# 331658260/Drone-YOLO

Measured on AMD Instinct MI355X. Metric: images/sec @640x640 Drone-YOLO-s, higher is better.
Workload: dtype fp16; 1 GPU; Drone-YOLO-s (yolov8s-p2-repvgg.yaml, nc=10) inference 640x640: layout+forward+decode+NMS, inputs resident in HBM; fp16 storage / fp32 accumulate (BASELINE config 2 names bf16: bf16 storage fails the IoU >= 0.999 bar - 0.995 - so the headline runs the 16-bit format that meets it; same MFMA rate, same bytes); batch_per_gpu=256, global_batch=256, parallelism=batch-split x1, no collective, hipgraph=True, streams=2, max_det=300

## Files before the change

### drone-yolo_amd/_lib.py

```python
from __future__ import annotations

import ctypes as C
import os

_HERE = os.path.dirname(os.path.abspath(__file__))
LIB_PATH = os.path.join(_HERE, "lib", "libdyolo.so")

DY_BF16, DY_F16, DY_F32, DY_FP8, DY_F16X2 = 0, 1, 2, 3, 4
DY_ACT_NONE, DY_ACT_SILU, DY_ACT_SILU_L2E = 0, 1, 2
DY_MAX_LEVELS = 8
DY_WLAYOUT_ROWS, DY_WLAYOUT_HALO3X3, DY_WLAYOUT_FRAG1X1 = 0, 1, 2

_vp, _i32, _f32, _i64 = C.c_void_p, C.c_int32, C.c_float, C.c_int64


class PackJob(C.Structure):
    _fields_ = [("w", C.c_void_p), ("s_co", C.c_int64), ("s_ci", C.c_int64), ("s_r", C.c_int64), ("s_q", C.c_int64),
                ("cout", C.c_int32), ("cin", C.c_int32), ("ksize", C.c_int32), ("transpose_flip", C.c_int32), ("cin_logical", C.c_int32),
                ("w_layout", C.c_int32), ("dst", C.c_void_p), ("dst_elems", C.c_int64)]


class ConvDesc(C.Structure):

    _fields_ = [
        ("x", _vp), ("w", _vp), ("bias", _vp), ("residual", _vp), ("y", _vp),
        ("batch", _i32), ("h", _i32), ("w_in", _i32), ("cin", _i32), ("ld_x", _i32),
        ("ho", _i32), ("wo", _i32), ("cout", _i32), ("ld_y", _i32), ("ld_res", _i32),
        ("ksize", _i32), ("stride", _i32), ("pad", _i32),
        ("groups", _i32), ("act", _i32), ("dtype", _i32), ("out_f32", _i32),
        ("k_pad", _i32), ("cout_pad", _i32), ("up2x", _i32),
        ("x2", _vp), ("ld_x2", _i32), ("cin_split", _i32), ("w_layout", _i32),
        ("w_scale", _vp), ("act_scale", _f32), ("bn_stats", _vp), ("y_dtype1", _i32),
        ("bnb_z", _vp), ("bnb_ld_z", _i32), ("bnb_act", _i32), ("bnb_mean", _vp), ("bnb_rstd", _vp), ("bnb_gamma", _vp), ("bnb_beta", _vp),
    ]


class BranchDesc(C.Structure):

    _fields_ = [
        ("x", _vp), ("w3", _vp), ("b3", _vp), ("w1", _vp), ("b1", _vp), ("out", _vp),
        ("batch", _i32), ("h", _i32), ("w", _i32), ("ld_x", _i32), ("c_in", _i32), ("c_mid", _i32), ("nc", _i32), ("reg_max", _i32),
        ("kind", _i32), ("dtype", _i32), ("anchors", _i32), ("anchor0", _i32),
        ("stride", _f32),
        ("nms_workspace", _vp), ("nms_workspace_bytes", _i64), ("conf_thres", _f32), ("classes_mask", _vp), ("act_l2e", _i32),
    ]


class DecodeDesc(C.Structure):

    _fields_ = [
        ("level", _vp * DY_MAX_LEVELS),
        ("h", _i32 * DY_MAX_LEVELS), ("w", _i32 * DY_MAX_LEVELS), ("ld", _i32 * DY_MAX_LEVELS),
        ("stride", _f32 * DY_MAX_LEVELS),
        ("n_levels", _i32), ("batch", _i32), ("nc", _i32), ("reg_max", _i32),
        ("out", _vp),
        ("nms_workspace", _vp), ("nms_workspace_bytes", _i64), ("conf_thres", _f32), ("classes_mask", _vp),
    ]


class HeadDecodeDesc(C.Structure):

    _fields_ = [
        ("x_box", _vp * DY_MAX_LEVELS), ("x_cls", _vp * DY_MAX_LEVELS),
        ("w_box", _vp * DY_MAX_LEVELS), ("w_cls", _vp * DY_MAX_LEVELS),
        ("b_box", _vp * DY_MAX_LEVELS), ("b_cls", _vp * DY_MAX_LEVELS),
        ("ld_box", _i32 * DY_MAX_LEVELS), ("ld_cls", _i32 * DY_MAX_LEVELS),
        ("h", _i32 * DY_MAX_LEVELS), ("w", _i32 * DY_MAX_LEVELS),
        ("stride", _f32 * DY_MAX_LEVELS),
        ("n_levels", _i32), ("batch", _i32), ("nc", _i32), ("reg_max", _i32),
        ("c_box", _i32), ("c_cls", _i32), ("dtype", _i32),
        ("out", _vp),
        ("nms_workspace", _vp), ("nms_workspace_bytes", _i64), ("conf_thres", _f32), ("classes_mask", _vp),
    ]


class NmsDesc(C.Structure):

    _fields_ = [
        ("pred", _vp),
        ("batch", _i32), ("nc", _i32), ("n_extra", _i32), ("anchors", _i32),
        ("conf_thres", _f32), ("iou_thres", _f32),
        ("max_det", _i32), ("max_nms", _i32),
        ("max_wh", _f32), ("agnostic", _i32),
        ("classes_mask", _vp),
        ("out", _vp), ("out_count", _vp), ("out_index", _vp),
        ("workspace", _vp), ("workspace_bytes", _i64), ("prefiltered", _i32), ("multi_label", _i32),
    ]


class LossDesc(C.Structure):

    _fields_ = [
        ("level", _vp * DY_MAX_LEVELS),
        ("h", _i32 * DY_MAX_LEVELS), ("w", _i32 * DY_MAX_LEVELS), ("ld", _i32 * DY_MAX_LEVELS),
        ("stride", _f32 * DY_MAX_LEVELS),
        ("n_levels", _i32), ("batch", _i32), ("nc", _i32), ("reg_max", _i32),
        ("gt", _vp), ("gmax", _i32), ("topk", _i32),
        ("alpha", _f32), ("beta", _f32), ("box_gain", _f32), ("cls_gain", _f32), ("dfl_gain", _f32),
        ("out", _vp), ("out_owner", _vp), ("workspace", _vp), ("workspace_bytes", _i64),
        ("grad_level", _vp * DY_MAX_LEVELS), ("ld_grad", _i32 * DY_MAX_LEVELS),
    ]


class C2fDesc(C.Structure):

    _fields_ = [
        ("x", _vp), ("x_lo", _vp), ("y", _vp), ("w_cv1", _vp), ("w_m_cv1", _vp), ("w_m_cv2", _vp), ("w_cv2", _vp), ("bias", _vp),
        ("batch", _i32), ("h", _i32), ("w", _i32), ("cin", _i32), ("cin_lo", _i32), ("hidden", _i32), ("cout", _i32),
        ("ld_x", _i32), ("ld_x_lo", _i32), ("ld_y", _i32), ("shortcut", _i32), ("dtype", _i32), ("act_l2e", _i32),
    ]


class Stem2Desc(C.Structure):

    _fields_ = [
        ("x", _vp), ("w0", _vp), ("b0", _vp), ("w1", _vp), ("b1", _vp), ("y", _vp),
        ("n", _i32), ("h", _i32), ("w", _i32), ("ld_y", _i32), ("act0", _i32), ("act1", _i32), ("dtype", _i32),
        ("w1_scale", _vp),
    ]


class BnDesc(C.Structure):

    _fields_ = [
        ("z", _vp), ("y", _vp), ("addend", _vp), ("dy", _vp), ("dz", _vp),
        ("rows", _i64),
        ("c", _i32), ("ld_z", _i32), ("ld_y", _i32), ("ld_add", _i32), ("ld_dy", _i32), ("ld_dz", _i32), ("dtype", _i32), ("act", _i32),
        ("gamma", _vp), ("beta", _vp), ("mean", _vp), ("rstd", _vp), ("running_mean", _vp), ("running_var", _vp),
        ("eps", _f32), ("momentum", _f32),
        ("dgamma", _vp), ("dbeta", _vp), ("workspace", _vp), ("workspace_bytes", _i64), ("partial_slabs", _i32),
    ]


SIGNATURES = {
    "dy_version": (_i32, []),
    "dy_last_error_string": (C.c_char_p, []),
    "dy_last_kernel_name": (C.c_char_p, []),
    "dy_dtype_size": (_i32, [_i32]),
    "dy_pack_conv_weights_table_bytes": (C.c_int64, [_i32]),
    "dy_pack_conv_weights_table": (_i32, [C.POINTER(PackJob), _i32, _i32, _vp, C.c_int64, C.POINTER(C.c_int32)]),
    "dy_pack_conv_weights_batched": (_i32, [_vp, _i32, _i32, _i32, _vp]),
    "dy_conv_k_pad": (_i32, [_i32, _i32, _i32]),
    "dy_conv_cout_pad": (_i32, [_i32]),
    "dy_conv2d_nhwc": (_i32, [C.POINTER(ConvDesc), _vp]),
    "dy_conv_stats_written": (_i32, []),
    "dy_c2f_fused_supported": (_i32, [_i32, _i32, _i32, _i32, _i32, _i32]),
    "dy_c2f_fused": (_i32, [C.POINTER(C2fDesc), _vp]),
    "dy_stem2_fused_supported": (_i32, [_i32, _i32, _i32, _i32, _i32, _i32]),
    "dy_stem2_fused": (_i32, [C.POINTER(Stem2Desc), _vp]),
    "dy_stem_conv3x3s2_nchw": (_i32, [_vp, _vp, _vp, _vp, _i32, _i32, _i32, _i32, _i32, _i32, _i32, _i32, _vp]),
    "dy_stem_conv3x3s2_nchw_u8": (_i32, [_vp, _f32, _vp, _vp, _vp, _i32, _i32, _i32, _i32, _i32, _i32, _i32, _i32, _vp]),
    "dy_nchw_f32_to_nhwc": (_i32, [_vp, _vp, _i32, _i32, _i32, _i32, _i32, _i32, _i32, _vp]),
    "dy_resize_bilinear_u8_nchw_f32": (_i32, [_vp, _vp, _i32, _i32, _i32, _i32, _i32, _i32, _vp]),
    "dy_scale_img_nchw_f32": (_i32, [_vp, _vp, _i32, _i32, _i32, _i32, _i32, _i32, _i32, _i32, _i32, _f32, _vp]),
    "dy_nhwc_to_nchw_f32": (_i32, [_vp, _vp, _i32, _i32, _i32, _i32, _i32, _i32, _vp]),
    "dy_upsample2x_nhwc": (_i32, [_vp, _vp, _i32, _i32, _i32, _i32, _i32, _i32, _i32, _vp]),
    "dy_copy_nhwc": (_i32, [_vp, _vp, _i32, _i32, _i32, _i32, _i32, _i32, _i32, _vp]),
    "dy_sppf_maxpool3": (_i32, [_vp, _vp, _vp, _vp, _i32, _i32, _i32, _i32, _i32, _i32, _i32, _vp]),
    "dy_detect_decode": (_i32, [C.POINTER(DecodeDesc), _vp]),
    "dy_detect_head_decode_supported": (_i32, [_i32, _i32, _i32, _i32, _i32]),
    "dy_detect_head_decode": (_i32, [C.POINTER(HeadDecodeDesc), _vp]),
    "dy_nms_workspace_bytes": (_i64, [_i32, _i32]),
    "dy_nms": (_i32, [C.POINTER(NmsDesc), _vp]),
    "dy_scale_boxes": (_i32, [_vp, _vp, _vp, _i32, _i32, _vp]),
    "dy_detection_loss_workspace_bytes": (_i64, [_i32, _i32, _i32, _i32]),
    "dy_conv2d_wgrad_nhwc": (_i32, [C.POINTER(ConvDesc), _vp, _i32, _vp, _vp]),
    "dy_conv2d_wgrad_nhwc_ws": (_i32, [C.POINTER(ConvDesc), _vp, _i32, _vp, _vp, C.c_int64, _vp]),
    "dy_conv2d_wgrad_workspace_bytes": (C.c_int64, [C.POINTER(ConvDesc), _i32]),
    "dy_quantize_fp8_nhwc": (_i32, [_vp, _vp, _i64, _i32, _i32, _i32, _i32, _f32, _vp]),
    "dy_pack_conv_weights": (_i32, [_vp, _i64, _i64, _i64, _i64, _i32, _i32, _i32, _i32, _i32, _vp, _i64, _i32, _i32, _vp]),
    "dy_detect_branch_fused_supported": (_i32, [_i32, _i32, _i32, _i32, _i32, _i32, _i32]),
    "dy_detect_branch_fused": (_i32, [C.POINTER(BranchDesc), _vp]),
    "dy_nms_reset_counts": (_i32, [_vp, _i32, _vp]),
    "dy_conv2d_grouped_bwd_nhwc": (_i32, [C.POINTER(ConvDesc), _vp, _i32, _vp, _vp, _vp, _i32, _vp, _i32, _vp]),
    "dy_colsum": (_i32, [_vp, _vp, _i64, _i32, _i32, _i32, _vp]),
    "dy_nchw_u8_to_nhwc": (_i32, [_vp, _vp, _i32, _i32, _i32, _i32, _i32, _i32, _f32, _i32, _vp]),
    "dy_letterbox_u8_to_nchw_f32": (_i32, [_vp, _vp, _i32, _i32, _i32, _i32, _i32, _i32, _i32, _i32, _i32, _i32, _f32, _vp]),
    "dy_tiles_u8_to_nchw_f32": (_i32, [_vp, _vp, _vp, _i32, _i32, _i32, _i32, _i32, _i32, _f32, _vp]),
    "dy_rows_to_pred": (_i32, [_vp, _vp, _vp, _vp, _i32, _i32, _i32, _vp]),
    "dy_upsample2x_bwd_nhwc": (_i32, [_vp, _vp, _i32, _i32, _i32, _i32, _i32, _i32, _i32, _vp]),
    "dy_maxpool_bwd_nhwc": (_i32, [_vp, _vp, _vp, _i32, _i32, _i32, _i32, _i32, _i32, _i32, _i32, _i32, _i32, _vp]),
    "dy_add_nhwc": (_i32, [_vp, _vp, _vp, _i64, _i32, _i32, _i32, _i32, _i32, _vp]),
    "dy_add_dilated2_nhwc": (_i32, [_vp, _vp, _i32, _i32, _i32, _i32, _i32, _i32, _i32, _i32, _i32, _vp]),
    "dy_head_grad_split": (_i32, [_vp, _i32, _i64, _i32, _i32, _i32, _vp, _vp, _i32, _vp, _i32, _i32, _vp]),
    "dy_sumsq_f32": (_i32, [_vp, _i64, _vp, _vp]),
    "dy_sgd_step": (_i32, [_vp, _vp, _vp, _i64, _f32, _f32, _f32, _i32, _i32, _vp, _f32, _vp, _vp]),
    "dy_adamw_step": (_i32, [_vp, _vp, _vp, _vp, _i64, _f32, _f32, _f32, _f32, _f32, _i32, _vp, _f32, _vp, _vp]),
    "dy_amp_update": (_i32, [_vp, _vp, _f32, _f32, _i32, _vp]),
    "dy_ema_update": (_i32, [_vp, _vp, _i64, _f32, _vp]),
    "dy_grad_sink_flush": (_i32, [_vp, _i32, _vp, _vp, _vp]),
    "dy_bn_workspace_bytes": (_i64, [_i32]),
    "dy_bn_train_fwd": (_i32, [C.POINTER(BnDesc), _vp]),
    "dy_bn_train_bwd": (_i32, [C.POINTER(BnDesc), _vp]),
    "dy_silu_fwd": (_i32, [_vp, _vp, _i64, _i32, _i32, _i32, _i32, _vp]),
    "dy_silu_bwd": (_i32, [_vp, _vp, _vp, _i64, _i32, _i32, _i32, _i32, _i32, _vp]),
    "dy_detection_loss": (_i32, [C.POINTER(LossDesc), _vp]),
}

_lib = None


class DyoloError(RuntimeError):
    """A libdyolo call returned a non-zero ``dy_status``."""


def lib() -> C.CDLL:
    global _lib
    if _lib is None:
        if not os.path.exists(LIB_PATH):
            raise ImportError(
                f"{LIB_PATH} not found: the HIP extension has not been built. Run "
                "`python -c 'import __graft_entry__ as g; g.build()'` or `make -C drone-yolo_amd/csrc`. "
                "There is no CPU / eager fallback for this path."
            )
        handle = C.CDLL(LIB_PATH)
        for name, (res, args) in SIGNATURES.items():
            fn = getattr(handle, name)
            fn.restype = res
            fn.argtypes = args
        _lib = handle
    return _lib


def check(rc: int, what: str = "libdyolo") -> None:
    if rc != 0:
        msg = lib().dy_last_error_string()
        raise DyoloError(f"{what} failed with status {rc}: {msg.decode() if msg else ''}")
```

### drone-yolo_amd/csrc/nms.hip

```cpp
#include "common_hip.h"
#include "nms_ws.h"

#pragma clang fp contract(off)

namespace dy {

typedef unsigned long long u64;

struct NmsArgs {
  const float* pred;
  int batch, nc, nch, A;
  float conf, iou;
  int max_det, max_nms;
  float max_wh;
  int agnostic;
  const uint8_t* cmask;
  float* out;
  int* out_count;
  int* out_index;
  int* counts;
  u64* keys;
  unsigned short* cls;
  int P;
  int SL;
  int multi;
  int cap;
};

__global__ __launch_bounds__(256) void nms_filter_kernel(const NmsArgs p) {
  const int lane = threadIdx.x & 63;
  const long long total = (long long)p.batch * p.A;
  const long long nthreads = (long long)gridDim.x * 256;
  const long long iters = (total + nthreads - 1) / nthreads;
  for (long long it = 0; it < iters; ++it) {
    const long long idx = it * nthreads + (long long)blockIdx.x * 256 + threadIdx.x;
    const bool in = idx < total;
    const int b = in ? (int)(idx / p.A) : 0;
    const int a = in ? (int)(idx - (long long)b * p.A) : 0;
    bool pass = false;
    float best = 0.f;
    int bj = 0;
    if (in) {
      const float* s = p.pred + ((size_t)b * p.nch + 4) * (size_t)p.A + a;
      best = s[0];
      for (int c = 1; c < p.nc; ++c) {
        const float v = s[(size_t)c * p.A];
        if (v > best) {
          best = v;
          bj = c;
        }
      }
      pass = best > p.conf;
      if (pass && p.cmask) pass = p.cmask[bj] != 0;
    }
    u64 todo = __ballot(pass);
    while (todo != 0ull) {
      const int leader = __ffsll((long long)todo) - 1;
      const int bb = __shfl(b, leader);
      const bool mine = pass && b == bb;
      const u64 m = __ballot(mine);
      int base = 0;
      if (lane == leader) base = atomicAdd(p.counts + bb, __popcll(m));
      base = __shfl(base, leader);
      if (mine) {
        const int pos = base + __popcll(m & ((1ull << lane) - 1ull));
        const unsigned bits = __float_as_uint(best);
        p.keys[(size_t)bb * p.P + pos] = ((u64)(~bits) << 32) | (u64)(unsigned)a;
        p.cls[(size_t)bb * p.A + a] = (unsigned short)bj;
      }
      todo &= ~m;
    }
  }
}

__global__ __launch_bounds__(256) void nms_filter_ml_kernel(const NmsArgs p) {
  const int lane = threadIdx.x & 63;
  const long long total = (long long)p.batch * p.A;
  const long long nthreads = (long long)gridDim.x * 256;
  const long long iters = (total + nthreads - 1) / nthreads;
  for (long long it = 0; it < iters; ++it) {
    const long long idx = it * nthreads + (long long)blockIdx.x * 256 + threadIdx.x;
    const bool in = idx < total;
    const int b = in ? (int)(idx / p.A) : 0;
    const int a = in ? (int)(idx - (long long)b * p.A) : 0;
    const float* s = p.pred + ((size_t)b * p.nch + 4) * (size_t)p.A + a;
    for (int c = 0; c < p.nc; ++c) {
      const float v = in ? s[(size_t)c * p.A] : 0.f;
      bool pass = in && v > p.conf;
      if (pass && p.cmask) pass = p.cmask[c] != 0;
      u64 todo = __ballot(pass);
      while (todo != 0ull) {
        const int leader = __ffsll((long long)todo) - 1;
        const int bb = __shfl(b, leader);
        const bool mine = pass && b == bb;
        const u64 m = __ballot(mine);
        int base = 0;
        if (lane == leader) base = atomicAdd(p.counts + bb, __popcll(m));
        base = __shfl(base, leader);
        if (mine) {
          const int pos = base + __popcll(m & ((1ull << lane) - 1ull));
          p.keys[(size_t)bb * p.P + pos] = ((u64)(~__float_as_uint(v)) << 32) | (u64)((unsigned)a * (unsigned)p.nc + (unsigned)c);
        }
        todo &= ~m;
      }
    }
  }
}

__device__ __forceinline__ bool iou_gt(float ix1, float iy1, float ix2, float iy2, float iarea, float jx1, float jy1,
                                       float jx2, float jy2, float jarea, float thr) {
  const float xx1 = fmaxf(ix1, jx1), yy1 = fmaxf(iy1, jy1);
  const float xx2 = fminf(ix2, jx2), yy2 = fminf(iy2, jy2);
  const float w = fmaxf(0.f, xx2 - xx1), h = fmaxf(0.f, yy2 - yy1);
  const float inter = w * h;
  const float ovr = inter / (iarea + jarea - inter);
  return ovr > thr;
}

__global__ __launch_bounds__(1024) void nms_suppress_kernel(const NmsArgs p) {
  extern __shared__ __attribute__((aligned(16))) unsigned char dyn_smem[];
  u64* skeys = reinterpret_cast<u64*>(dyn_smem);
  float* kept = reinterpret_cast<float*>(dyn_smem + (size_t)p.SL * 8);
  const int b = blockIdx.x;
  const int tid = threadIdx.x;
  int n = p.counts[b];
  if (n > p.cap) n = p.cap;
  u64* gkeys = p.keys + (size_t)b * p.P;

  int P2 = 1;
  while (P2 < n) P2 <<= 1;
  const bool in_lds = P2 <= p.SL;
  auto bitonic = [&](auto* keys) {
    for (int k = 2; k <= P2; k <<= 1) {
      for (int j = k >> 1; j > 0; j >>= 1) {
        for (int t = tid; t < (P2 >> 1); t += 1024) {
          const int i = ((t & ~(j - 1)) << 1) | (t & (j - 1));
          const int ixj = i | j;
          const u64 x = keys[i], y = keys[ixj];
          const bool up = (i & k) == 0;
          if ((x > y) == up) {
            keys[i] = y;
            keys[ixj] = x;
          }
        }
        __syncthreads();
      }
    }
  };
  if (in_lds) {
    for (int i = tid; i < P2; i += 1024) skeys[i] = i < n ? gkeys[i] : ~0ull;
    __syncthreads();
    if (n > 1) bitonic(skeys);
  } else {
    for (int i = n + tid; i < P2; i += 1024) gkeys[i] = ~0ull;
    __syncthreads();
    bitonic(gkeys);
  }
  if (tid >= 64) return;

  const int lane = tid;
  const int nn = n < p.max_nms ? n : p.max_nms;
  float* kx1 = kept;
  float* ky1 = kept + p.max_det;
  float* kx2 = kept + 2 * p.max_det;
  float* ky2 = kept + 3 * p.max_det;
  float* kar = kept + 4 * p.max_det;
  const float* pr = p.pred + (size_t)b * p.nch * (size_t)p.A;
  float* outb = p.out + (size_t)b * p.max_det * 6;
  int nk = 0;
  for (int c0 = 0; c0 < nn && nk < p.max_det; c0 += 64) {
    const int i = c0 + lane;
    bool alive = i < nn;
    float x1 = 0.f, y1 = 0.f, x2 = 0.f, y2 = 0.f, ox1 = 0.f, oy1 = 0.f, ox2 = 0.f, oy2 = 0.f, area = 0.f, score = 0.f;
    int anchor = 0, cls = 0;
    if (alive) {
      const u64 key = in_lds ? skeys[i] : gkeys[i];
      anchor = (int)(unsigned)(key & 0xffffffffull);
      score = __uint_as_float(~(unsigned)(key >> 32));
      if (p.multi) {
        cls = anchor % p.nc;
        anchor = anchor / p.nc;
      } else {
        cls = (int)p.cls[(size_t)b * p.A + anchor];
      }
      const float cx = pr[anchor], cy = pr[(size_t)p.A + anchor];
      const float hw = pr[(size_t)2 * p.A + anchor] / 2.f, hh = pr[(size_t)3 * p.A + anchor] / 2.f;
      x1 = cx - hw;
      y1 = cy - hh;
      x2 = cx + hw;
      y2 = cy + hh;
      const float off = p.agnostic ? 0.f : (float)cls * p.max_wh;
      ox1 = x1 + off;
      oy1 = y1 + off;
      ox2 = x2 + off;
      oy2 = y2 + off;
      area = (ox2 - ox1) * (oy2 - oy1);
      for (int k = 0; k < nk; ++k)
        if (iou_gt(kx1[k], ky1[k], kx2[k], ky2[k], kar[k], ox1, oy1, ox2, oy2, area, p.iou)) {
          alive = false;
          break;
        }
    }
    u64 am = __ballot(alive);
    while (am != 0ull) {
      const int t = __ffsll((long long)am) - 1;
      auto bcast = [&](float v) { return __uint_as_float(__builtin_amdgcn_readlane(__float_as_uint(v), t)); };
      const float tx1 = bcast(ox1), ty1 = bcast(oy1), tx2 = bcast(ox2), ty2 = bcast(oy2), tar = bcast(area);
      if (lane == t) {
        kx1[nk] = ox1;
        ky1[nk] = oy1;
        kx2[nk] = ox2;
        ky2[nk] = oy2;
        kar[nk] = area;
        float* o = outb + (size_t)nk * 6;
        o[0] = x1;
        o[1] = y1;
        o[2] = x2;
        o[3] = y2;
        o[4] = score;
        o[5] = (float)cls;
        if (p.out_index) p.out_index[(size_t)b * p.max_det + nk] = anchor;
        alive = false;
      }
      ++nk;
      if (nk >= p.max_det) break;
      if (alive && lane > t && iou_gt(tx1, ty1, tx2, ty2, tar, ox1, oy1, ox2, oy2, area, p.iou)) alive = false;
      am = __ballot(alive);
    }
  }
  for (int r = nk * 6 + lane; r < p.max_det * 6; r += 64) outb[r] = 0.f;
  if (p.out_index)
    for (int r = nk + lane; r < p.max_det; r += 64) p.out_index[(size_t)b * p.max_det + r] = -1;
  if (lane == 0) p.out_count[b] = nk;
}

__global__ __launch_bounds__(256) void scale_boxes_kernel(float* __restrict__ boxes, const int* __restrict__ counts,
                                                          const float* __restrict__ params, int batch, int max_det) {
  const int idx = blockIdx.x * 256 + threadIdx.x;
  if (idx >= batch * max_det) return;
  const int b = idx / max_det, r = idx - b * max_det;
  if (r >= counts[b]) return;
  const float gain = params[b * 5], px = params[b * 5 + 1], py = params[b * 5 + 2];
  const float cw = params[b * 5 + 3], ch = params[b * 5 + 4];
  float* o = boxes + (size_t)idx * 6;
  o[0] = fminf(fmaxf((o[0] - px) / gain, 0.f), cw);
  o[1] = fminf(fmaxf((o[1] - py) / gain, 0.f), ch);
  o[2] = fminf(fmaxf((o[2] - px) / gain, 0.f), cw);
  o[3] = fminf(fmaxf((o[3] - py) / gain, 0.f), ch);
}

static inline int next_pow2(int v) { return nms_next_pow2(v); }
static inline size_t align_up(size_t v, size_t a) { return nms_align_up(v, a); }

}

using namespace dy;

extern "C" int64_t dy_nms_workspace_bytes(int32_t batch, int32_t anchors) {
  if (batch <= 0 || anchors <= 0) return -1;
  return (int64_t)nms_ws_bytes(batch, anchors);
}

extern "C" int32_t dy_nms(const dy_nms_desc* d, dy_stream_t stream) {
  DY_REQUIRE(d && d->pred && d->out && d->out_count && d->workspace, DY_ERR_INVALID_ARG, "dy_nms: null pointer");
  DY_REQUIRE(d->batch > 0 && d->nc > 0 && d->anchors > 0 && d->n_extra >= 0, DY_ERR_INVALID_ARG, "dy_nms: bad dims");
  DY_REQUIRE(d->nc <= 65535, DY_ERR_UNSUPPORTED, "dy_nms: nc %d > 65535", d->nc);
  DY_REQUIRE(d->conf_thres >= 0.f && d->conf_thres <= 1.f && d->iou_thres >= 0.f && d->iou_thres <= 1.f,
             DY_ERR_INVALID_ARG, "dy_nms: thresholds must be in [0,1] (utils/ops.py:233-234)");
  DY_REQUIRE(d->max_det >= 1 && d->max_det <= 4096 && d->max_nms >= 1, DY_ERR_INVALID_ARG, "dy_nms: max_det must be in [1,4096]");
  const bool multi = d->multi_label != 0 && d->nc > 1;
  DY_REQUIRE(!multi || (long long)d->anchors * d->nc < (1ll << 30), DY_ERR_UNSUPPORTED, "dy_nms: multi_label with anchors * nc >= 2^30");
  DY_REQUIRE(!(multi && d->prefiltered), DY_ERR_UNSUPPORTED, "dy_nms: the fused candidate filter is single-label; multi_label filters here");
  const int wcap = multi ? d->anchors * d->nc : d->anchors;
  const int64_t need = dy_nms_workspace_bytes(d->batch, wcap);
  DY_REQUIRE(d->workspace_bytes >= need, DY_ERR_WORKSPACE, "dy_nms: workspace %lld < %lld bytes", (long long)d->workspace_bytes,
             (long long)need);
  DY_REQUIRE(aligned16(d->workspace), DY_ERR_INVALID_ARG, "dy_nms: workspace not 16-byte aligned");
  hipStream_t st = reinterpret_cast<hipStream_t>(stream);

  NmsArgs a{};
  a.pred = d->pred;
  a.batch = d->batch;
  a.nc = d->nc;
  a.nch = 4 + d->nc + d->n_extra;
  a.A = d->anchors;
  a.conf = d->conf_thres;
  a.iou = d->iou_thres;
  a.max_det = d->max_det;
  a.max_nms = d->max_nms;
  a.max_wh = d->max_wh;
  a.agnostic = d->agnostic;
  a.cmask = d->classes_mask;
  a.out = d->out;
  a.out_count = d->out_count;
  a.out_index = d->out_index;
  const NmsWs w = nms_ws_layout(d->workspace, d->batch, wcap);
  a.multi = multi ? 1 : 0;
  a.cap = wcap;
  a.P = w.P;
  a.counts = w.counts;
  a.keys = reinterpret_cast<u64*>(w.keys);
  a.cls = w.cls;
  a.SL = a.P < 16384 ? a.P : 16384;

  if (!d->prefiltered) {
    zero_async(a.counts, (size_t)d->batch * 4, st);
    const long long total = (long long)d->batch * d->anchors;
    long long blocks = (total + 255) / 256;
    if (blocks > 4096) blocks = 4096;
    if (multi) hipLaunchKernelGGL(nms_filter_ml_kernel, dim3((unsigned)blocks), dim3(256), 0, st, a);
    else hipLaunchKernelGGL(nms_filter_kernel, dim3((unsigned)blocks), dim3(256), 0, st, a);
    const int rc = check_launch(multi ? "nms_filter_ml_kernel" : "nms_filter_kernel");
    if (rc != DY_OK) return rc;
  }
  const size_t smem = (size_t)a.SL * 8 + align_up((size_t)d->max_det * 5 * 4, 16);
  static const hipError_t attr_once = hipFuncSetAttribute((const void*)nms_suppress_kernel, hipFuncAttributeMaxDynamicSharedMemorySize, 160 * 1024);
  (void)attr_once;
  hipLaunchKernelGGL(nms_suppress_kernel, dim3((unsigned)d->batch), dim3(1024), smem, st, a);
  return check_launch("nms_suppress_kernel");
}

extern "C" int32_t dy_scale_boxes(float* boxes, const int32_t* counts, const float* params, int32_t batch,
                                  int32_t max_det, dy_stream_t stream) {
  DY_REQUIRE(boxes && counts && params, DY_ERR_INVALID_ARG, "dy_scale_boxes: null pointer");
  DY_REQUIRE(batch > 0 && max_det > 0, DY_ERR_INVALID_ARG, "dy_scale_boxes: bad dims");
  const int total = batch * max_det;
  hipLaunchKernelGGL(scale_boxes_kernel, dim3((unsigned)((total + 255) / 256)), dim3(256), 0,
                     reinterpret_cast<hipStream_t>(stream), boxes, counts, params, batch, max_det);
  return check_launch("scale_boxes_kernel");
}
```

### include/dyolo.h

```cpp
#ifndef DYOLO_H_
#define DYOLO_H_

#include <stdint.h>

#ifdef __cplusplus
extern "C" {
#endif

#define DYOLO_VERSION_MAJOR 0
#define DYOLO_VERSION_MINOR 1

typedef void* dy_stream_t;

typedef enum dy_status {
  DY_OK = 0,
  DY_ERR_INVALID_ARG = -1,
  DY_ERR_UNSUPPORTED = -2,
  DY_ERR_LAUNCH = -3,
  DY_ERR_WORKSPACE = -4
} dy_status;

typedef enum dy_dtype { DY_BF16 = 0, DY_F16 = 1, DY_F32 = 2, DY_FP8 = 3, DY_F16X2 = 4 } dy_dtype;
typedef enum dy_act { DY_ACT_NONE = 0, DY_ACT_SILU = 1, DY_ACT_SILU_L2E = 2 } dy_act;
typedef enum dy_wlayout { DY_WLAYOUT_ROWS = 0, DY_WLAYOUT_HALO3X3 = 1, DY_WLAYOUT_FRAG1X1 = 2 } dy_wlayout;


int32_t dy_version(void);
const char* dy_last_error_string(void);
const char* dy_last_kernel_name(void);
int32_t dy_dtype_size(int32_t dtype);

typedef struct dy_conv_desc {
  const void* x;
  const void* w;
  const float* bias;
  const void* residual;
  void* y;
  int32_t batch, h, w_in, cin, ld_x;
  int32_t ho, wo, cout, ld_y, ld_res;
  int32_t ksize, stride, pad;
  int32_t groups;
  int32_t act;
  int32_t dtype;
  int32_t out_f32;
  int32_t k_pad, cout_pad;
  int32_t up2x;
  const void* x2;
  int32_t ld_x2, cin_split;
  int32_t w_layout;
  const float* w_scale;
  float act_scale;
  double* bn_stats;
  int32_t y_dtype1;
  const void* bnb_z;
  int32_t bnb_ld_z, bnb_act;
  const float* bnb_mean;
  const float* bnb_rstd;
  const float* bnb_gamma;
  const float* bnb_beta;
} dy_conv_desc;

int32_t dy_quantize_fp8_nhwc(const void* src, void* dst, int64_t rows, int32_t c, int32_t ld_src, int32_t ld_dst, int32_t src_dtype, float act_scale,
                             dy_stream_t stream);
int32_t dy_pack_conv_weights(const float* w, int64_t s_co, int64_t s_ci, int64_t s_r, int64_t s_q, int32_t cout, int32_t cin, int32_t ksize,
                             int32_t transpose_flip, int32_t cin_logical, void* dst, int64_t dst_elems, int32_t dtype, int32_t w_layout, dy_stream_t stream);
typedef struct dy_pack_job {
  const float* w;
  int64_t s_co, s_ci, s_r, s_q;
  int32_t cout, cin, ksize, transpose_flip, cin_logical, w_layout;
  void* dst;
  int64_t dst_elems;
} dy_pack_job;
int64_t dy_pack_conv_weights_table_bytes(int32_t n_jobs);
int32_t dy_pack_conv_weights_table(const dy_pack_job* jobs, int32_t n_jobs, int32_t dtype, void* table_host, int64_t table_bytes, int32_t* total_blocks);
int32_t dy_pack_conv_weights_batched(const void* table_dev, int32_t n_jobs, int32_t total_blocks, int32_t dtype, dy_stream_t stream);
int32_t dy_conv_k_pad(int32_t cin, int32_t ksize, int32_t dtype);
int32_t dy_conv_cout_pad(int32_t cout);
int32_t dy_conv2d_nhwc(const dy_conv_desc* d, dy_stream_t stream);
int32_t dy_conv_stats_written(void);

typedef struct dy_branch_desc {
  const void* x;
  const void* w3;
  const float* b3;
  const void* w1;
  const float* b1;
  float* out;
  int32_t batch, h, w, ld_x, c_in, c_mid, nc, reg_max, kind, dtype, anchors, anchor0;
  float stride;
  void* nms_workspace;
  int64_t nms_workspace_bytes;
  float conf_thres;
  const uint8_t* classes_mask;
  int32_t act_l2e;
} dy_branch_desc;
int32_t dy_detect_branch_fused_supported(int32_t c_in, int32_t c_mid, int32_t c_out, int32_t kind, int32_t nc, int32_t reg_max, int32_t dtype);
int32_t dy_detect_branch_fused(const dy_branch_desc* d, dy_stream_t stream);
int32_t dy_nms_reset_counts(void* nms_workspace, int32_t batch, dy_stream_t stream);

typedef struct dy_c2f_desc {
  const void* x;
  const void* x_lo;
  void* y;
  const void* w_cv1;
  const void* w_m_cv1;
  const void* w_m_cv2;
  const void* w_cv2;
  const float* bias;
  int32_t batch, h, w, cin, cin_lo, hidden, cout, ld_x, ld_x_lo, ld_y, shortcut, dtype;
  int32_t act_l2e;
} dy_c2f_desc;
int32_t dy_c2f_fused_supported(int32_t cin, int32_t cin_lo, int32_t hidden, int32_t cout, int32_t n_bottlenecks, int32_t dtype);
int32_t dy_c2f_fused(const dy_c2f_desc* d, dy_stream_t stream);

int32_t dy_stem_conv3x3s2_nchw(const float* x, const void* w, const float* bias, void* y, int32_t n, int32_t cin,
                               int32_t h, int32_t w_in, int32_t cout, int32_t ld_y, int32_t act, int32_t dtype,
                               dy_stream_t stream);

int32_t dy_stem_conv3x3s2_nchw_u8(const uint8_t* x, float divisor, const void* w, const float* bias, void* y, int32_t n, int32_t cin,
                                  int32_t h, int32_t w_in, int32_t cout, int32_t ld_y, int32_t act, int32_t dtype, dy_stream_t stream);

typedef struct dy_stem2_desc {
  const float* x;
  const void* w0;
  const float* b0;
  const void* w1;
  const float* b1;
  void* y;
  int32_t n, h, w, ld_y, act0, act1, dtype;
  const float* w1_scale;
} dy_stem2_desc;
int32_t dy_stem2_fused_supported(int32_t cin, int32_t c0, int32_t c1, int32_t h, int32_t w, int32_t dtype);
int32_t dy_stem2_fused(const dy_stem2_desc* d, dy_stream_t stream);

int32_t dy_letterbox_u8_to_nchw_f32(const uint8_t* src, float* dst, int32_t n, int32_t h0, int32_t w0, int32_t new_w, int32_t new_h,
                                    int32_t top, int32_t left, int32_t hn, int32_t wn, int32_t swap_rb, float pad_value,
                                    dy_stream_t stream);

int32_t dy_resize_bilinear_u8_nchw_f32(const uint8_t* src, float* dst, int32_t n, int32_t c, int32_t h, int32_t w, int32_t ho, int32_t wo, dy_stream_t stream);
int32_t dy_scale_img_nchw_f32(const float* src, float* dst, int32_t n, int32_t c, int32_t h, int32_t w, int32_t hs, int32_t ws, int32_t ho, int32_t wo,
                              int32_t flip_lr, float pad, dy_stream_t stream);

int32_t dy_tiles_u8_to_nchw_f32(const uint8_t* frame, const int32_t* offsets_yx, float* dst, int32_t k, int32_t hf, int32_t wf, int32_t th,
                                int32_t tw, int32_t swap_rb, float pad_value, dy_stream_t stream);
int32_t dy_rows_to_pred(const float* rows, const int32_t* counts, const int32_t* offsets_yx, float* pred, int32_t k, int32_t max_det,
                        int32_t nc, dy_stream_t stream);


int32_t dy_nchw_f32_to_nhwc(const float* src, void* dst, int32_t n, int32_t c, int32_t h, int32_t w,
                            int32_t c_pad, int32_t ld_dst, int32_t dtype, dy_stream_t stream);

int32_t dy_nchw_u8_to_nhwc(const uint8_t* src, void* dst, int32_t n, int32_t c, int32_t h, int32_t w, int32_t c_pad,
                           int32_t ld_dst, float divisor, int32_t dtype, dy_stream_t stream);

int32_t dy_nhwc_to_nchw_f32(const void* src, float* dst, int32_t n, int32_t c, int32_t h, int32_t w,
                            int32_t ld_src, int32_t src_dtype, dy_stream_t stream);

int32_t dy_upsample2x_nhwc(const void* src, void* dst, int32_t n, int32_t h, int32_t w, int32_t c,
                           int32_t ld_src, int32_t ld_dst, int32_t dtype, dy_stream_t stream);

int32_t dy_copy_nhwc(const void* src, void* dst, int32_t n, int32_t h, int32_t w, int32_t c,
                     int32_t ld_src, int32_t ld_dst, int32_t dtype, dy_stream_t stream);

int32_t dy_sppf_maxpool3(const void* x, void* y1, void* y2, void* y3, int32_t n, int32_t h, int32_t w,
                         int32_t c, int32_t ld, int32_t k, int32_t dtype, dy_stream_t stream);

#define DY_MAX_LEVELS 8
typedef struct dy_decode_desc {
  const float* level[DY_MAX_LEVELS];
  int32_t h[DY_MAX_LEVELS], w[DY_MAX_LEVELS], ld[DY_MAX_LEVELS];
  float stride[DY_MAX_LEVELS];
  int32_t n_levels, batch, nc, reg_max;
  float* out;
  void* nms_workspace;
  int64_t nms_workspace_bytes;
  float conf_thres;
  const uint8_t* classes_mask;
} dy_decode_desc;
int32_t dy_detect_decode(const dy_decode_desc* d, dy_stream_t stream);

typedef struct dy_head_decode_desc {
  const void* x_box[DY_MAX_LEVELS];
  const void* x_cls[DY_MAX_LEVELS];
  const void* w_box[DY_MAX_LEVELS];
  const void* w_cls[DY_MAX_LEVELS];
  const float* b_box[DY_MAX_LEVELS];
  const float* b_cls[DY_MAX_LEVELS];
  int32_t ld_box[DY_MAX_LEVELS], ld_cls[DY_MAX_LEVELS], h[DY_MAX_LEVELS], w[DY_MAX_LEVELS];
  float stride[DY_MAX_LEVELS];
  int32_t n_levels, batch, nc, reg_max, c_box, c_cls, dtype;
  float* out;
  void* nms_workspace;
  int64_t nms_workspace_bytes;
  float conf_thres;
  const uint8_t* classes_mask;
} dy_head_decode_desc;
int32_t dy_detect_head_decode_supported(int32_t c_box, int32_t c_cls, int32_t nc, int32_t reg_max, int32_t dtype);
int32_t dy_detect_head_decode(const dy_head_decode_desc* d, dy_stream_t stream);

typedef struct dy_nms_desc {
  const float* pred;
  int32_t batch, nc, n_extra, anchors;
  float conf_thres, iou_thres;
  int32_t max_det, max_nms;
  float max_wh;
  int32_t agnostic;
  const uint8_t* classes_mask;
  float* out;
  int32_t* out_count;
  int32_t* out_index;
  void* workspace;
  int64_t workspace_bytes;
  int32_t prefiltered;
  int32_t multi_label;
} dy_nms_desc;
int64_t dy_nms_workspace_bytes(int32_t batch, int32_t anchors);
int32_t dy_nms(const dy_nms_desc* d, dy_stream_t stream);

int32_t dy_scale_boxes(float* boxes, const int32_t* counts, const float* params, int32_t batch,
                       int32_t max_det, dy_stream_t stream);

typedef struct dy_loss_desc {
  const float* level[DY_MAX_LEVELS];
  int32_t h[DY_MAX_LEVELS], w[DY_MAX_LEVELS], ld[DY_MAX_LEVELS];
  float stride[DY_MAX_LEVELS];
  int32_t n_levels, batch, nc, reg_max;
  const float* gt;
  int32_t gmax, topk;
  float alpha, beta, box_gain, cls_gain, dfl_gain;
  float* out;
  int32_t* out_owner;
  void* workspace;
  int64_t workspace_bytes;
  float* grad_level[DY_MAX_LEVELS];
  int32_t ld_grad[DY_MAX_LEVELS];
} dy_loss_desc;
int64_t dy_detection_loss_workspace_bytes(int32_t batch, int32_t anchors, int32_t gmax, int32_t topk);
int32_t dy_detection_loss(const dy_loss_desc* d, dy_stream_t stream);

int32_t dy_conv2d_wgrad_nhwc(const dy_conv_desc* d, const void* dz, int32_t ld_dz, float* dw, dy_stream_t stream);
int32_t dy_conv2d_wgrad_nhwc_ws(const dy_conv_desc* d, const void* dz, int32_t ld_dz, float* dw, void* workspace, int64_t workspace_bytes,
                                dy_stream_t stream);
int64_t dy_conv2d_wgrad_workspace_bytes(const dy_conv_desc* d, int32_t ld_dz);
int32_t dy_colsum(const void* z, float* out, int64_t rows, int32_t c, int32_t ld, int32_t dtype, dy_stream_t stream);
int32_t dy_conv2d_grouped_bwd_nhwc(const dy_conv_desc* d, const void* dz, int32_t ld_dz, const float* w_oihw, float* dw_oihw, void* dx, int32_t ld_dx,
                                   const void* dx_accumulate, int32_t ld_acc, dy_stream_t stream);

typedef struct dy_bn_desc {
  const void* z;
  void* y;
  const void* addend;
  const void* dy;
  void* dz;
  int64_t rows;
  int32_t c, ld_z, ld_y, ld_add, ld_dy, ld_dz, dtype, act;
  const float* gamma;
  const float* beta;
  float* mean;
  float* rstd;
  float* running_mean;
  float* running_var;
  float eps, momentum;
  float* dgamma;
  float* dbeta;
  void* workspace;
  int64_t workspace_bytes;
  int32_t partial_slabs;
} dy_bn_desc;
int64_t dy_bn_workspace_bytes(int32_t c);
int32_t dy_bn_train_fwd(const dy_bn_desc* d, dy_stream_t stream);
int32_t dy_bn_train_bwd(const dy_bn_desc* d, dy_stream_t stream);
int32_t dy_silu_fwd(const void* u, void* y, int64_t rows, int32_t c, int32_t ld_u, int32_t ld_y, int32_t dtype, dy_stream_t stream);
int32_t dy_silu_bwd(const void* u, const void* dy, void* du, int64_t rows, int32_t c, int32_t ld_u, int32_t ld_dy, int32_t ld_du,
                    int32_t dtype, dy_stream_t stream);

int32_t dy_upsample2x_bwd_nhwc(const void* g, void* dx, int32_t n, int32_t h, int32_t w, int32_t c, int32_t ld_g, int32_t ld_dx,
                               int32_t dtype, dy_stream_t stream);
int32_t dy_maxpool_bwd_nhwc(const void* x, const void* g_out, void* g_in, int32_t n, int32_t h, int32_t w, int32_t c, int32_t ld_x,
                            int32_t ld_go, int32_t ld_gi, int32_t k, int32_t accumulate, int32_t dtype, dy_stream_t stream);
int32_t dy_add_dilated2_nhwc(const void* t, void* dx, int32_t n, int32_t h, int32_t w, int32_t H2, int32_t W2, int32_t c, int32_t ld_t, int32_t ld_dx,
                             int32_t dtype, dy_stream_t stream);
int32_t dy_head_grad_split(const float* g, int32_t ld_g, int64_t rows, int32_t nb, int32_t nc, int32_t ncp, const float* scale, void* dzb, int32_t ld_b,
                           void* dzc, int32_t ld_c, int32_t dtype, dy_stream_t stream);
int32_t dy_add_nhwc(const void* a, const void* b, void* out, int64_t rows, int32_t c, int32_t ld_a, int32_t ld_b, int32_t ld_o,
                    int32_t dtype, dy_stream_t stream);

int32_t dy_sumsq_f32(const float* g, int64_t n, double* out, dy_stream_t stream);
int32_t dy_sgd_step(float* p, const float* grad, float* buf, int64_t n, float lr, float momentum, float weight_decay, int32_t nesterov,
                    int32_t first_step, const double* grad_sumsq, float max_norm, const float* amp_state, dy_stream_t stream);
int32_t dy_adamw_step(float* p, const float* grad, float* m, float* v, int64_t n, float lr, float beta1, float beta2, float eps,
                      float weight_decay, int32_t step, const double* grad_sumsq, float max_norm, const float* amp_state, dy_stream_t stream);
int32_t dy_amp_update(float* amp_state, const double* grad_sumsq, float growth_factor, float backoff_factor, int32_t growth_interval, dy_stream_t stream);
int32_t dy_ema_update(float* ema, const float* p, int64_t n, float decay, dy_stream_t stream);
int32_t dy_grad_sink_flush(const int64_t* entries, int32_t n_entries, float* grad, float* sink, dy_stream_t stream);

#ifdef __cplusplus
}
#endif
#endif
```

Measured before the change: 20060 images/sec.

## Add wave-parallel small-candidate NMS kernel with ballot-based greedy suppression

Adds a 256-thread NMS kernel for images with at most 2048 candidates. It sorts the candidates in LDS, then processes them in 64-wide chunks, using wave ballots and readlane broadcasts to build an intra-chunk IoU bitmask and resolve greedy suppression without per-candidate block syncs. The existing 1024-thread kernel now exits early for small counts and is skipped entirely when the workspace cap fits the small path. This trades an extra launch plus duplicated logic for lower sync and occupancy cost on the common case, where each image has few candidates.

```diff
diff --git a/drone-yolo_amd/_lib.py b/drone-yolo_amd/_lib.py
--- a/drone-yolo_amd/_lib.py
+++ b/drone-yolo_amd/_lib.py
@@ -162,6 +162,7 @@
     "dy_detect_head_decode": (_i32, [C.POINTER(HeadDecodeDesc), _vp]),
     "dy_nms_workspace_bytes": (_i64, [_i32, _i32]),
     "dy_nms": (_i32, [C.POINTER(NmsDesc), _vp]),
+    "dy_nms_small_cap": (_i32, []),
     "dy_scale_boxes": (_i32, [_vp, _vp, _vp, _i32, _i32, _vp]),
     "dy_detection_loss_workspace_bytes": (_i64, [_i32, _i32, _i32, _i32]),
     "dy_conv2d_wgrad_nhwc": (_i32, [C.POINTER(ConvDesc), _vp, _i32, _vp, _vp]),
diff --git a/drone-yolo_amd/csrc/nms.hip b/drone-yolo_amd/csrc/nms.hip
--- a/drone-yolo_amd/csrc/nms.hip
+++ b/drone-yolo_amd/csrc/nms.hip
@@ -117,6 +117,148 @@
   return ovr > thr;
 }
 
+constexpr int NMS_SMALL_CAP = 2048;
+constexpr int NMS_SMALL_THREADS = 256;
+constexpr int NMS_SMALL_WAVES = NMS_SMALL_THREADS / 64;
+constexpr int NMS_SMALL_FIXED_LDS = NMS_SMALL_CAP * 8 + 64 * 8 + NMS_SMALL_WAVES * 8;
+
+static inline size_t nms_small_lds_bytes(int max_det) { return (size_t)NMS_SMALL_FIXED_LDS + (size_t)max_det * 20; }
+
+struct NmsCand {
+  float cx, cy, w, h, score;
+  int anchor, cls;
+};
+
+__device__ __forceinline__ NmsCand nms_small_fetch(const NmsArgs& p, const u64* skeys, const float* pr, int b, int i, int nn) {
+  NmsCand c{0.f, 0.f, 0.f, 0.f, 0.f, 0, 0};
+  if (i < nn) {
+    const u64 key = skeys[i];
+    c.anchor = (int)(unsigned)(key & 0xffffffffull);
+    c.score = __uint_as_float(~(unsigned)(key >> 32));
+    if (p.multi) {
+      c.cls = c.anchor % p.nc;
+      c.anchor = c.anchor / p.nc;
+    } else {
+      c.cls = (int)p.cls[(size_t)b * p.A + c.anchor];
+    }
+    c.cx = pr[c.anchor];
+    c.cy = pr[(size_t)p.A + c.anchor];
+    c.w = pr[(size_t)2 * p.A + c.anchor];
+    c.h = pr[(size_t)3 * p.A + c.anchor];
+  }
+  return c;
+}
+
+__device__ __forceinline__ u64 nms_uniform64(u64 v) {
+  const unsigned lo = (unsigned)__builtin_amdgcn_readfirstlane((int)(unsigned)v);
+  const unsigned hi = (unsigned)__builtin_amdgcn_readfirstlane((int)(unsigned)(v >> 32));
+  return ((u64)hi << 32) | (u64)lo;
+}
+
+__global__ __launch_bounds__(NMS_SMALL_THREADS) void nms_small_kernel(const NmsArgs p) {
+  extern __shared__ __attribute__((aligned(16))) unsigned char dyn_smem[];
+  const int b = blockIdx.x;
+  int n = p.counts[b];
+  if (n > p.cap) n = p.cap;
+  if (n > NMS_SMALL_CAP) return;
+  u64* skeys = reinterpret_cast<u64*>(dyn_smem);
+  u64* rows = skeys + NMS_SMALL_CAP;
+  u64* verdict = rows + 64;
+  float4* kbox = reinterpret_cast<float4*>(dyn_smem + NMS_SMALL_FIXED_LDS);
+  float* kar = reinterpret_cast<float*>(kbox + p.max_det);
+  const int tid = threadIdx.x;
+  const int lane = tid & 63;
+  const int wave = __builtin_amdgcn_readfirstlane(tid >> 6);
+  const u64* gkeys = p.keys + (size_t)b * p.P;
+
+  int P2 = 1;
+  while (P2 < n) P2 <<= 1;
+  for (int i = tid; i < P2; i += NMS_SMALL_THREADS) skeys[i] = i < n ? gkeys[i] : ~0ull;
+  __syncthreads();
+  for (int k = 2; k <= P2; k <<= 1) {
+    for (int j = k >> 1; j > 0; j >>= 1) {
+      for (int t = tid; t < (P2 >> 1); t += NMS_SMALL_THREADS) {
+        const int i = ((t & ~(j - 1)) << 1) | (t & (j - 1));
+        const int ixj = i | j;
+        const u64 x = skeys[i], y = skeys[ixj];
+        const bool up = (i & k) == 0;
+        if ((x > y) == up) {
+          skeys[i] = y;
+          skeys[ixj] = x;
+        }
+      }
+      __syncthreads();
+    }
+  }
+
+  const int nn = n < p.max_nms ? n : p.max_nms;
+  const float* pr = p.pred + (size_t)b * p.nch * (size_t)p.A;
+  float* outb = p.out + (size_t)b * p.max_det * 6;
+  const u64 lane_bit = 1ull << lane;
+  int nk = 0;
+  NmsCand nxt = nms_small_fetch(p, skeys, pr, b, lane, nn);
+  for (int c0 = 0; c0 < nn && nk < p.max_det; c0 += 64) {
+    const NmsCand c = nxt;
+    nxt = nms_small_fetch(p, skeys, pr, b, c0 + 64 + lane, nn);
+    const bool in = c0 + lane < nn;
+    const float hw = c.w / 2.f, hh = c.h / 2.f;
+    const float x1 = c.cx - hw, y1 = c.cy - hh, x2 = c.cx + hw, y2 = c.cy + hh;
+    const float off = p.agnostic ? 0.f : (float)c.cls * p.max_wh;
+    const float ox1 = x1 + off, oy1 = y1 + off, ox2 = x2 + off, oy2 = y2 + off;
+    const float area = (ox2 - ox1) * (oy2 - oy1);
+    bool sup = false;
+    for (int k = wave; k < nk; k += NMS_SMALL_WAVES) {
+      const float4 kb = kbox[k];
+      sup |= iou_gt(kb.x, kb.y, kb.z, kb.w, kar[k], ox1, oy1, ox2, oy2, area, p.iou);
+    }
+    const u64 sm = __ballot(sup);
+    u64 myrow = 0ull;
+    for (int r = 0; r < 16; ++r) {
+      const int i = wave * 16 + r;
+      auto bcast = [&](float v) { return __uint_as_float(__builtin_amdgcn_readlane(__float_as_uint(v), i)); };
+      const u64 m = __ballot(iou_gt(bcast(ox1), bcast(oy1), bcast(ox2), bcast(oy2), bcast(area), ox1, oy1, ox2, oy2, area, p.iou));
+      if (lane == r) myrow = m;
+    }
+    if (lane < 16) rows[wave * 16 + lane] = myrow;
+    if (lane == 0) verdict[wave] = sm;
+    __syncthreads();
+    u64 dead = 0ull;
+    for (int w = 0; w < NMS_SMALL_WAVES; ++w) dead |= verdict[w];
+    const u64 row = rows[lane];
+    const unsigned row_lo = (unsigned)row, row_hi = (unsigned)(row >> 32);
+    u64 am = __ballot(in) & ~nms_uniform64(dead);
+    u64 km = 0ull;
+    int cnt = 0;
+    while (am != 0ull) {
+      const int t = __ffsll((long long)am) - 1;
+      km |= 1ull << t;
+      ++cnt;
+      if (nk + cnt >= p.max_det) break;
+      const u64 rt = ((u64)(unsigned)__builtin_amdgcn_readlane((int)row_hi, t) << 32) | (u64)(unsigned)__builtin_amdgcn_readlane((int)row_lo, t);
+      am &= ~(rt | (1ull << t));
+    }
+    if (wave == 0 && (km & lane_bit) != 0ull) {
+      const int at = nk + __popcll(km & (lane_bit - 1ull));
+      kbox[at] = make_float4(ox1, oy1, ox2, oy2);
+      kar[at] = area;
+      float* o = outb + (size_t)at * 6;
+      o[0] = x1;
+      o[1] = y1;
+      o[2] = x2;
+      o[3] = y2;
+      o[4] = c.score;
+      o[5] = (float)c.cls;
+      if (p.out_index) p.out_index[(size_t)b * p.max_det + at] = c.anchor;
+    }
+    nk += cnt;
+    __syncthreads();
+  }
+  for (int r = nk * 6 + tid; r < p.max_det * 6; r += NMS_SMALL_THREADS) outb[r] = 0.f;
+  if (p.out_index)
+    for (int r = nk + tid; r < p.max_det; r += NMS_SMALL_THREADS) p.out_index[(size_t)b * p.max_det + r] = -1;
+  if (tid == 0) p.out_count[b] = nk;
+}
+
 __global__ __launch_bounds__(1024) void nms_suppress_kernel(const NmsArgs p) {
   extern __shared__ __attribute__((aligned(16))) unsigned char dyn_smem[];
   u64* skeys = reinterpret_cast<u64*>(dyn_smem);
@@ -125,6 +267,7 @@
   const int tid = threadIdx.x;
   int n = p.counts[b];
   if (n > p.cap) n = p.cap;
+  if (n <= NMS_SMALL_CAP) return;
   u64* gkeys = p.keys + (size_t)b * p.P;
 
   int P2 = 1;
@@ -313,12 +456,20 @@
     const int rc = check_launch(multi ? "nms_filter_ml_kernel" : "nms_filter_kernel");
     if (rc != DY_OK) return rc;
   }
+  static const hipError_t attr_small = hipFuncSetAttribute((const void*)nms_small_kernel, hipFuncAttributeMaxDynamicSharedMemorySize, 160 * 1024);
+  (void)attr_small;
+  hipLaunchKernelGGL(nms_small_kernel, dim3((unsigned)d->batch), dim3(NMS_SMALL_THREADS), nms_small_lds_bytes(d->max_det), st, a);
+  const int rc = check_launch("nms_small_kernel");
+  if (rc != DY_OK) return rc;
+  if (wcap <= NMS_SMALL_CAP) return DY_OK;
   const size_t smem = (size_t)a.SL * 8 + align_up((size_t)d->max_det * 5 * 4, 16);
   static const hipError_t attr_once = hipFuncSetAttribute((const void*)nms_suppress_kernel, hipFuncAttributeMaxDynamicSharedMemorySize, 160 * 1024);
   (void)attr_once;
   hipLaunchKernelGGL(nms_suppress_kernel, dim3((unsigned)d->batch), dim3(1024), smem, st, a);
   return check_launch("nms_suppress_kernel");
 }
+
+extern "C" int32_t dy_nms_small_cap(void) { return NMS_SMALL_CAP; }
 
 extern "C" int32_t dy_scale_boxes(float* boxes, const int32_t* counts, const float* params, int32_t batch,
                                   int32_t max_det, dy_stream_t stream) {
diff --git a/include/dyolo.h b/include/dyolo.h
--- a/include/dyolo.h
+++ b/include/dyolo.h
@@ -216,6 +216,7 @@
 } dy_nms_desc;
 int64_t dy_nms_workspace_bytes(int32_t batch, int32_t anchors);
 int32_t dy_nms(const dy_nms_desc* d, dy_stream_t stream);
+int32_t dy_nms_small_cap(void);
 
 int32_t dy_scale_boxes(float* boxes, const int32_t* counts, const float* params, int32_t batch,
                        int32_t max_det, dy_stream_t stream);
```

Result: faster. 20260 images/sec, median of 6 (+1.0%).
